# carlmoore256/MAAVSS

Measured on AMD Instinct MI355X. Metric: train clips/sec (16-frame×224² + 512-pt STFT) at 1/2/4/8 MI355X; mask-MSE vs ref, higher is better.
Workload: dtype f16; 1 GPU; batch=32/GPU, 16 frames 224x224, 512-pt STFT, ViT-S/8 attention extraction (f16 MFMA operands, f32 accumulate) + STFT + AV_Fusion_Model_Frames fwd+bwd (16-bit MFMA conv, f32 accumulate) + Adam; global_batch=32, frames=16, framesize=224, fft_len=512, parallelism=dp1, streams=2 (extraction of batch i+1 under the training step of batch i), avse_spatial_match=adaptive, vit_weights=random-init (no network), vit=f16, vit_gelu=f32, vit_qkv_ln=pre, vit_attention=f16, conv_fwd=f16, linear_lstm=f32 (split-K by f32 atomics), batchnorm=per-rank, grad_all_reduce=f32 wire, per-module buckets in backward order

## Files before the change

### include/maavss.h

```cpp
#ifndef MAAVSS_H
#define MAAVSS_H
#include <stdint.h>
#ifdef __cplusplus
extern "C" {
#endif

#define MAAVSS_ABI_VERSION 400
const char* maavss_last_error(void);
int maavss_version(void);
const char* maavss_arch(void);

int maavss_stft_fwd(const float* audio, int64_t batch, int64_t length, int64_t audio_stride, const float* window,
                    int n_fft, int hop, int n_frames, int n_bins_out, float* y, float* x, const float* noise,
                    float sigma, uint64_t seed, float* clip_absmax, void* stream);
int maavss_stft_normalise(float* y, float* x, const float* noise, const float* clip_absmax, int64_t batch,
                          int n_frames, int n_bins_out, float sigma, uint64_t seed, void* stream);

int maavss_istft(const float* spec, int64_t batch, int n_frames, int n_bins_in, const float* window, int n_fft, int hop,
                 int normalized, float* frames_ws, float* audio, int64_t audio_stride, void* stream);

int maavss_set_deterministic(int on);
int maavss_get_deterministic(void);
int maavss_set_deterministic_workspace(float* ws, int64_t bytes, void* stream);
int maavss_gemm_f32(const float* A, int64_t lda, int transA, const float* B, int64_t ldb, int transB, float* C,
// ... 114 lines not shown
int maavss_vit_patchify(const float* frames, void* a, int64_t n_frames, int H, int W, int dtype, void* stream);
int maavss_vit_gemm(const void* A, int lda, const void* W, const float* bias, const float* table, int period, void* C,
                    int ldc, int64_t M, int N, int K, int epilogue, int qscale_cols, float qscale, int dtype, void* stream);
int maavss_vit_layernorm(const float* x, const float* gamma, const float* beta, void* y, int64_t rows, int dim,
                         float eps, int dtype, void* stream);
int maavss_vit_panel_gemm(const float* X, const void* A, int lda, const float* ln_gamma, const float* ln_beta,
                          float ln_eps, const void* W, const float* bias, void* C, int ldc, int64_t c_rows, int64_t M,
                          int N, int epilogue, int qscale_cols, float qscale, int dtype, void* stream);
int maavss_vit_ws_gemm(const void* A, int lda, int64_t a_rows, const void* W, const float* bias, void* C, int ldc,
                       int64_t c_rows, int64_t M, int N, int epilogue, int qscale_cols, float qscale, void* xn_out,
                       const float* ln_gamma, const float* ln_beta, float ln_eps, int dtype, void* stream);
int maavss_vit_ws_gemm_ln(const float* X, int64_t x_rows, const float* row_stats, const float* ln_gamma, const float* ln_beta,
                          float ln_eps, const void* W, const float* bias, void* C, int ldc, int64_t c_rows, int64_t M, int N,
                          int qscale_cols, float qscale, int dtype, void* stream);
int maavss_vit_ws_gemm_ln_post(const float* X, int64_t x_rows, const float* row_stats, const float* col_sums, float ln_eps, const void* W,
                               const float* bias, void* C, int ldc, int64_t c_rows, int64_t M, int N, int qscale_cols, float qscale, int dtype,
                               void* stream);
int maavss_vit_gemm_stats(const void* A, int lda, const void* W, const float* bias, const float* table, int period, void* C,
                          int ldc, int64_t M, int N, int K, int epilogue, int qscale_cols, float qscale, float* row_stats,
                          int dtype, void* stream);
int maavss_vit_attn(const void* qkv, void* out, int frames, int ntok, int heads, int ld_qkv, int ld_out, int dtype,
                    void* stream);
int maavss_vit_cls_attn(const void* qkv, float* att, int frames, int ntok, int heads, int ld_qkv, int dtype, void* stream);
int64_t maavss_vit_attn_mx_ws_bytes(int64_t rows);
int maavss_vit_qkv_mx(const void* qkv, void* ws, int64_t rows, int ld_qkv, int dtype, void* stream);
int maavss_vit_attn_mx(const void* ws, void* out, int frames, int ntok, int heads, int ld_out, int dtype, void* stream);
int maavss_vit_ws_gemm_ln_mx(const float* X, int64_t x_rows, const float* row_stats, const float* ln_gamma, const float* ln_beta,
                             float ln_eps, const void* W, const float* bias, void* mx_ws, int64_t M, int qscale_cols, float qscale,
                             int dtype, void* stream);
int maavss_vit_attn_maps(const float* att, float* out, float* ws, int64_t n_frames, int heads, int H, int W,
                         int clip_frames, int attn_diff , void* stream);
int maavss_vit_attn_maps_checked(const float* att, float* out, float* ws, int64_t n_frames, int heads, int H, int W,
                                 int clip_frames, int attn_diff, int32_t* nonfinite_flag, void* stream);

int maavss_adaptive_pool_fwd(const float* x, float* out, int B, int H, int W, int C, int Ho, int Wo, int64_t os_b,
                             int64_t os_p, int64_t os_c, void* stream);
int maavss_adaptive_pool_bwd(const float* dout, float* dx, int B, int H, int W, int C, int Ho, int Wo, int64_t os_b,
                             int64_t os_p, int64_t os_c, void* stream);

int64_t maavss_video_transform_ws_bytes(int64_t F, int clip_frames, int H0, int W0, int S, int antialias, int autocontrast);
int maavss_video_transform(const void* src, const int32_t* boxes, const int32_t* host_boxes, float* out, void* ws, int64_t ws_bytes,
                           int64_t F, int clip_frames, int H0, int W0, int S, float mean0, float mean1, float mean2, float std0,
                           float std1, float std2, int antialias, int autocontrast, void* stream);

int maavss_vit_attn_maps_pass1(const float* att, float* small, float* fmax, int64_t n_frames, int heads, int n,
                               int32_t* nonfinite_flag, void* stream);
// ... 15 lines not shown
```

### maavss_amd/csrc/vit_attn.hip

```cpp
#include <type_traits>
#include "mma.h"

#define ATT_D 64
#define ATT_QT 128
#define ATT_KT 64
#define ATT_THR 5.0f
#ifdef MAAVSS_ATTN_ABLATE
#include <stdlib.h>
#define ABL(bit) ((ABLM >> (bit)) & 1)
#else
#define ABL(bit) 0
#endif

__device__ __forceinline__ float fast_exp2(float x) { return __builtin_amdgcn_exp2f(x); }

template <int MODE, int ABLM = 0>
__global__ __launch_bounds__(256) __attribute__((amdgpu_waves_per_eu(3, 3))) void vit_attn_kernel(
    const bf16_t* __restrict__ qkv, bf16_t* __restrict__ out, int ntok, int ld_qkv, int ld_out, int dim, int heads, int qblocks,
    int ngroups) {
  __shared__ __attribute__((aligned(16))) bf16_t Ks[2][ATT_KT * ATT_D];
  __shared__ __attribute__((aligned(16))) bf16_t Vs[2][ATT_KT * ATT_D];
  const int tid = threadIdx.x, lane = tid & 63, wv = tid >> 6, r = lane & 31, h = lane >> 5;
  const int xcd = blockIdx.x & 7, slot = blockIdx.x >> 3;
  const int group = (slot / qblocks) * 8 + xcd;
// ... 187 lines not shown
    if (last_half) tile(ntiles - 1, std::true_type{}, std::integral_constant<int, 1>{});
    else tile(ntiles - 1, std::true_type{}, std::integral_constant<int, 2>{});
  }
  {
    float la, lb;
    lane_swap32(lrow, la, lb);
    const float inv = 1.f / (la + lb);
    const int qr = q0 + r;
    if (qr < ntok) {
      bf16_t* op = out + (row0 + qr) * ld_out + head * ATT_D + 4 * h;
#pragma unroll
      for (int db = 0; db < 2; ++db)
#pragma unroll
        for (int g = 0; g < 4; ++g) {
          uint2 u;
          u.x = pack2<MODE>(o[db][4 * g] * inv, o[db][4 * g + 1] * inv);
          u.y = pack2<MODE>(o[db][4 * g + 2] * inv, o[db][4 * g + 3] * inv);
          *reinterpret_cast<uint2*>(op + 32 * db + 8 * g) = u;
        }
    }
  }
}

template <int MODE>
__global__ __launch_bounds__(256) void vit_cls_attn_kernel(const bf16_t* __restrict__ qkv, float* __restrict__ att, int ntok,
                                                           int ld_qkv, int dim) {
  extern __shared__ float sc[];
  __shared__ float qv[ATT_D];
  __shared__ float red[4];
  const int tid = threadIdx.x, head = blockIdx.x, frame = blockIdx.y;
  const int64_t row0 = (int64_t)frame * ntok;
  if (tid < ATT_D) qv[tid] = up16<MODE>(qkv[row0 * ld_qkv + head * ATT_D + tid]);
  __syncthreads();
  float mx = -1e30f;
  for (int j = tid; j < ntok; j += 256) {
    const bf16_t* kp = qkv + (row0 + j) * ld_qkv + dim + head * ATT_D;
    float acc = 0.f;
#pragma unroll
    for (int c = 0; c < 8; ++c) {
      const uint4 u = *reinterpret_cast<const uint4*>(kp + c * 8);
      const unsigned w[4] = {u.x, u.y, u.z, u.w};
#pragma unroll
      for (int e = 0; e < 4; ++e) {
        acc = fmaf(up16<MODE>((unsigned short)(w[e] & 0xffffu)), qv[c * 8 + 2 * e], acc);
        acc = fmaf(up16<MODE>((unsigned short)(w[e] >> 16)), qv[c * 8 + 2 * e + 1], acc);
      }
    }
    sc[j] = acc;
    mx = fmaxf(mx, acc);
  }
  mx = wave_max(mx);
  if ((tid & 63) == 0) red[tid >> 6] = mx;
  __syncthreads();
  mx = fmaxf(fmaxf(red[0], red[1]), fmaxf(red[2], red[3]));
  __syncthreads();
  float sum = 0.f;
  for (int j = tid; j < ntok; j += 256) {
    const float p = exp2f(sc[j] - mx);
    sc[j] = p;
    sum += p;
  }
  sum = wave_sum(sum);
  if ((tid & 63) == 0) red[tid >> 6] = sum;
  __syncthreads();
  const float inv = 1.f / (red[0] + red[1] + red[2] + red[3]);
  float* ap = att + ((int64_t)frame * gridDim.x + head) * (ntok - 1);
  for (int j = tid + 1; j < ntok; j += 256) ap[j - 1] = sc[j] * inv;
}

extern "C" int maavss_vit_attn(const void* qkv, void* out, int frames, int ntok, int heads, int ld_qkv, int ld_out, int dtype,
                               void* stream) {
  MAAVSS_CHECK_ARG(qkv && out && frames > 0 && ntok > 0, "vit_attn: bad arguments");
  MAAVSS_CHECK_ARG(heads >= 1 && ld_qkv >= 3 * heads * ATT_D && ld_out >= heads * ATT_D && ld_qkv % 8 == 0 && ld_out % 4 == 0,
                   "vit_attn: bad layout");
  MAAVSS_CHECK_ARG(dtype == MODE_BF16 || dtype == MODE_F16, "vit_attn: dtype must be 0 (bf16) or 2 (f16)");
  const int qblocks = cdiv(ntok, ATT_QT), ngroups = frames * heads;
  const int nblocks = cdiv(ngroups, 8) * 8 * qblocks;
  const bf16_t* q = (const bf16_t*)qkv;
  bf16_t* o = (bf16_t*)out;
  hipStream_t st = (hipStream_t)stream;
#ifdef MAAVSS_ATTN_ABLATE
  {
    const char* e = getenv("MAAVSS_ATTN_ABL");
    const int m = e ? atoi(e) : 0;
#define ABL_CASE(M) case M: hipLaunchKernelGGL((vit_attn_kernel<MODE_F16, M>), dim3(nblocks), dim3(256), 0, st, q, o, ntok, ld_qkv, ld_out, heads * ATT_D, heads, qblocks, ngroups); break;
    switch (m) { ABL_CASE(0) ABL_CASE(1) ABL_CASE(2) ABL_CASE(3) ABL_CASE(4) ABL_CASE(7) ABL_CASE(8) ABL_CASE(15) ABL_CASE(16) ABL_CASE(32) ABL_CASE(48) ABL_CASE(64) ABL_CASE(128) ABL_CASE(192) ABL_CASE(207) ABL_CASE(240)
      default: MAAVSS_CHECK_ARG(false, "vit_attn (ablation build): mask %d not instantiated", m); }
#undef ABL_CASE
    MAAVSS_LAUNCH_CHECK("vit_attn_kernel");
    return MAAVSS_OK;
  }
#endif
  if (dtype == MODE_F16)
    hipLaunchKernelGGL(vit_attn_kernel<MODE_F16>, dim3(nblocks), dim3(256), 0, st, q, o, ntok, ld_qkv, ld_out, heads * ATT_D, heads, qblocks, ngroups);
  else
    hipLaunchKernelGGL(vit_attn_kernel<MODE_BF16>, dim3(nblocks), dim3(256), 0, st, q, o, ntok, ld_qkv, ld_out, heads * ATT_D, heads, qblocks, ngroups);
  MAAVSS_LAUNCH_CHECK("vit_attn_kernel");
  return MAAVSS_OK;
}

extern "C" int maavss_vit_cls_attn(const void* qkv, float* att, int frames, int ntok, int heads, int ld_qkv, int dtype, void* stream) {
  MAAVSS_CHECK_ARG(qkv && att && frames > 0 && ntok > 1, "vit_cls_attn: bad arguments");
  MAAVSS_CHECK_ARG((size_t)ntok * 4 <= 60 * 1024, "vit_cls_attn: too many tokens for the LDS score buffer");
  MAAVSS_CHECK_ARG(dtype == MODE_BF16 || dtype == MODE_F16, "vit_cls_attn: dtype must be 0 (bf16) or 2 (f16)");
  if (dtype == MODE_F16)
    hipLaunchKernelGGL(vit_cls_attn_kernel<MODE_F16>, dim3(heads, frames), dim3(256), ntok * sizeof(float), (hipStream_t)stream,
                       (const bf16_t*)qkv, att, ntok, ld_qkv, heads * ATT_D);
  else
    hipLaunchKernelGGL(vit_cls_attn_kernel<MODE_BF16>, dim3(heads, frames), dim3(256), ntok * sizeof(float), (hipStream_t)stream,
                       (const bf16_t*)qkv, att, ntok, ld_qkv, heads * ATT_D);
  MAAVSS_LAUNCH_CHECK("vit_cls_attn_kernel");
  return MAAVSS_OK;
}
```

### maavss_amd/csrc/vit_ws_gemm.hip

```cpp
#include <type_traits>
#include <stdlib.h>
#include "mma.h"
#include "vit_epilogue.h"
#include "vit_mx.h"

#define WS_K 384
#define WS_BM 64
#define WS_WAVES 12
#define WS_THREADS (WS_WAVES * 64)
#define WS_SLICE (WS_WAVES * 32)
#define WS_BUFS 2
#define WS_PANEL_BYTES (WS_BM * WS_K * 2)

struct WsArgs {
  const bf16_t* A;
  const float* X;
  const float* row_stats;
  const bf16_t* W;
  const float* bias;
  void* C;
  bf16_t* XN;
  const float* ln_g;
  const float* ln_b;
  float ln_eps;
  int M, N, ldc;
  int qscale_cols;
  float qscale;
  int ns;
  int groups_per_xcd;
  int panels;
  MxImages mx;
};

#ifdef WS_STAMP
__device__ unsigned long long ws_stamps[256 * WS_WAVES * 8];
extern "C" int maavss_ws_stamps_read(unsigned long long* host, int clear) {
  if (hipMemcpyFromSymbol(host, HIP_SYMBOL(ws_stamps), sizeof(ws_stamps)) != hipSuccess) return 1;
  if (clear) { static unsigned long long z[256 * WS_WAVES * 8]; if (hipMemcpyToSymbol(HIP_SYMBOL(ws_stamps), z, sizeof(z)) != hipSuccess) return 1; }
  return 0;
}
#define WS_T(i) { const unsigned long long t_ = __builtin_amdgcn_s_memtime(); st_acc[i] += t_ - st_last; st_last = t_; }
#else
#define WS_T(i)
#endif

template <int EPI, int LN, int MODE, int SH>
__global__ __launch_bounds__(WS_THREADS) void vit_ws_gemm_kernel(WsArgs g) {
  static_assert(SH == 32 || SH == 16, "MFMA shape");
  static_assert(SH == 32 || EPI != 3, "the MX epilogue is built on the 32x32 accumulator layout");
  constexpr bool LN_POST = LN == 5;
  constexpr bool LN_OUT = LN == 1 || LN == 3, LN_IN = LN == 2 || LN == 4 || LN_POST, AFF = LN == 1 || LN == 2;
  static_assert(LN >= 0 && LN <= 5, "LN variant");
  static_assert(!LN_POST || (SH == 16 && EPI == 0), "LayerNorm after the product: 16x16x32 form, 16-bit epilogue");
  static_assert(!LN_OUT || EPI == 2, "LayerNorm of the output rows comes with the residual epilogue");
  static_assert(!LN_IN || EPI == 0 || EPI == 3, "LayerNorm on the way in is wired for the attn.qkv epilogues");
  static_assert(EPI != 3 || LN_IN, "the MX epilogue is wired for attn.qkv (LayerNorm on the way in)");
  extern __shared__ __attribute__((aligned(16))) char smem[];
  char* panels_lds = smem;
  float* bias_lds = reinterpret_cast<float*>(smem + WS_BUFS * WS_PANEL_BYTES);
  float* gam_lds = bias_lds + WS_SLICE;
  float* bet_lds = gam_lds + WS_SLICE;
  float2* stat_lds = reinterpret_cast<float2*>(bet_lds + WS_SLICE);
  const int tid = threadIdx.x, lane = tid & 63, wv = tid >> 6, r32 = lane & 31, half = lane >> 5;
  const int xcd = blockIdx.x & 7, slot = blockIdx.x >> 3;
  if (slot >= g.groups_per_xcd * g.ns) return;
  const int slice = slot % g.ns, group = xcd * g.groups_per_xcd + slot / g.ns, ngroups = 8 * g.groups_per_xcd;
  const int p0 = (int)((int64_t)g.panels * group / ngroups), p1 = (int)((int64_t)g.panels * (group + 1) / ngroups);
  if (p0 >= p1) return;
  const int n0 = slice * WS_SLICE + wv * 32;
#ifdef MAAVSS_WS_ABL
  constexpr int abl = MAAVSS_WS_ABL;
#else
  constexpr int abl = 0;
#endif

  typedef unsigned u32x4 __attribute__((ext_vector_type(4)));
  u32x4 stg0, stg1, stg2, stg3;
#define WS_FETCH(p)                                                                                               \
// ... 32 lines not shown
    int ln_ = lane;                                                                                               \
    asm volatile("" : "+v"(ln_));                                                                                 \
    char* dst_ = panels_lds + (buf) * WS_PANEL_BYTES;                                                             \
    WS_DEPOSIT_HALF_ONE(part, 0, stg0) WS_DEPOSIT_HALF_ONE(part, 1, stg1)                                         \
  }
  float4 st01;
  float2 st2;
#define WS_FETCH_X(hp, with_stats, srow)                                                                           \
  {                                                                                                               \
    const char* src_ = reinterpret_cast<const char*>(g.X) + (int64_t)(hp) * WS_PANEL_BYTES + (wv * 256 + lane) * 16; \
    if (with_stats) {                                                                                             \
      const char* sp_ = reinterpret_cast<const char*>(g.row_stats) + (int64_t)(srow) * 24;                         \
      asm volatile("global_load_dwordx4 %0, %6, off\n\tglobal_load_dwordx4 %1, %6, off offset:1024\n\t"            \
                   "global_load_dwordx4 %2, %6, off offset:2048\n\tglobal_load_dwordx4 %3, %6, off offset:3072\n\t" \
                   "global_load_dwordx4 %4, %7, off\n\tglobal_load_dwordx2 %5, %7, off offset:16"                  \
                   : "=&v"(stg0), "=&v"(stg1), "=&v"(stg2), "=&v"(stg3), "=&v"(st01), "=&v"(st2) : "v"(src_), "v"(sp_) : "memory"); \
    } else {                                                                                                      \
      asm volatile("global_load_dwordx4 %0, %4, off\n\tglobal_load_dwordx4 %1, %4, off offset:1024\n\t"            \
                   "global_load_dwordx4 %2, %4, off offset:2048\n\tglobal_load_dwordx4 %3, %4, off offset:3072"    \
                   : "=&v"(stg0), "=&v"(stg1), "=&v"(stg2), "=&v"(stg3) : "v"(src_) : "memory");                   \
    }                                                                                                             \
  }
  float2* table_lds = stat_lds;
  auto merge_stats = [&](const float4& a, const float2& b) __attribute__((always_inline)) {
    const float mean = (a.x + a.z + b.x) * (1.f / 3.f);
    const float d0 = a.x - mean, d1 = a.z - mean, d2 = b.x - mean;
    const float m2 = (a.y + a.w + b.y) + 128.f * (d0 * d0 + d1 * d1 + d2 * d2);
    return make_float2(mean, rsqrtf(m2 * (1.f / WS_K) + g.ln_eps));
  };
  auto deposit_ln_one = [&](char* dst, const float2* tab, int part, int i, const u32x4& raw, int ln) __attribute__((always_inline)) {
    const int q = (wv * 4 + i) * 64 + ln, r = q / 96, c4 = q - r * 96, rr = 32 * part + r;
    float2 ms = make_float2(0.f, 0.f);
    if constexpr (!LN_POST) ms = tab[rr];
    const float4 v = __builtin_bit_cast(float4, raw);
    uint2 o;
    if constexpr (LN_POST) {
      o = make_uint2(pack2<MODE>(v.x, v.y), pack2<MODE>(v.z, v.w));
    } else if constexpr (AFF) {
      const float4 gg = *reinterpret_cast<const float4*>(gam_lds + 4 * c4), bb = *reinterpret_cast<const float4*>(bet_lds + 4 * c4);
      o = make_uint2(pack2<MODE>((v.x - ms.x) * ms.y * gg.x + bb.x, (v.y - ms.x) * ms.y * gg.y + bb.y),
                     pack2<MODE>((v.z - ms.x) * ms.y * gg.z + bb.z, (v.w - ms.x) * ms.y * gg.w + bb.w));
    } else {
      o = make_uint2(pack2<MODE>((v.x - ms.x) * ms.y, (v.y - ms.x) * ms.y), pack2<MODE>((v.z - ms.x) * ms.y, (v.w - ms.x) * ms.y));
    }
    *reinterpret_cast<uint2*>(dst + rr * (WS_K * 2) + (((c4 >> 1) ^ (rr & 15)) << 4) + (c4 & 1) * 8) = o;
  };
#define WS_DEPOSIT_LN(buf, tab, part)                                                                             \
  {                                                                                                               \
    int ln_ = lane;                                                                                               \
    asm volatile("" : "+v"(ln_));                                                                                 \
    char* dst_ = panels_lds + (buf) * WS_PANEL_BYTES;                                                             \
    deposit_ln_one(dst_, tab, part, 0, stg0, ln_); deposit_ln_one(dst_, tab, part, 1, stg1, ln_);                 \
    deposit_ln_one(dst_, tab, part, 2, stg2, ln_); deposit_ln_one(dst_, tab, part, 3, stg3, ln_);                 \
  }
  constexpr bool SPLIT = EPI == 2;
  if constexpr (!LN_IN) WS_FETCH(p0)

#ifndef WS16_LN_SPLITCOLS
#define WS16_LN_SPLITCOLS 0
#endif
  constexpr bool F32OUT = EPI == 2 && (!LN_OUT || WS16_LN_SPLITCOLS);
  constexpr int CSTEP = F32OUT ? 16 : 4;
  const int j16 = lane & 15, g16 = lane >> 4;
  const int cbase16 = F32OUT ? 4 * g16 : 8 * g16;
  bf16x8 w[24];
  if constexpr (SH == 32) {
    const int q = r32 >> 3, h = (r32 >> 2) & 1, r = r32 & 3;
    const bf16_t* wp = g.W + (int64_t)(n0 + 16 * (q >> 1) + 8 * h + 4 * (q & 1) + r) * WS_K + 8 * half;
#pragma unroll
    for (int kb = 0; kb < 24; ++kb) w[kb] = *reinterpret_cast<const bf16x8*>(wp + kb * 16);
  } else {
#pragma unroll
    for (int b = 0; b < 2; ++b) {
      const int col = F32OUT ? 16 * b + j16 : 8 * (j16 >> 2) + 4 * b + (j16 & 3);
      const bf16_t* wp = g.W + (int64_t)(n0 + col) * WS_K + 8 * g16;
#pragma unroll
      for (int ks = 0; ks < 12; ++ks) w[12 * b + ks] = *reinterpret_cast<const bf16x8*>(wp + ks * 32);
    }
  }
  if (tid < WS_SLICE) {
    bias_lds[tid] = g.bias[slice * WS_SLICE + tid];
    if constexpr (AFF) { gam_lds[tid] = g.ln_g[tid]; bet_lds[tid] = g.ln_b[tid]; }
    if constexpr (LN_POST) gam_lds[tid] = g.ln_g[slice * WS_SLICE + tid];
  }
  if constexpr (!LN_IN) {
    WS_WAIT_FETCH(0)
    WS_DEPOSIT(0)
  } else {
    if (wv < 2 && p0 + wv < p1) {
      int row = (p0 + wv) * WS_BM + lane;
      row = row < g.M ? row : g.M - 1;
      const float* sp = g.row_stats + (int64_t)row * 6;
      table_lds[wv * WS_BM + lane] = merge_stats(*reinterpret_cast<const float4*>(sp), *reinterpret_cast<const float2*>(sp + 4));
    }
    __syncthreads();
#pragma unroll 1
    for (int part = 0; part < 2; ++part) {
      WS_FETCH_X(2 * p0 + part, false, 0)
      WS_WAIT_FETCH(0)
      WS_DEPOSIT_LN(0, table_lds, part)
    }
  }
  const int frag_r = r32 * (WS_K * 2) + ((half ^ (r32 & 1)) << 4), frag_x = (r32 & 14) << 4;
  const int frag16_r = j16 * (WS_K * 2) + ((g16 ^ (j16 & 3)) << 4), frag16_x = (j16 & 12) << 4;
  const float scale = ((EPI == 0 || EPI == 3) && slice * WS_SLICE < g.qscale_cols) ? g.qscale : 1.f;
  const bool vslice = EPI == 3 && slice == 2;

  constexpr int S = EPI == 2 ? (LN_OUT ? (SH == 16 && WS16_LN_SPLITCOLS ? 24 : 20) : 16) : 4;
  int it = 0;
#ifdef WS_STAMP
  unsigned long long st_acc[6] = {0, 0, 0, 0, 0, 0}, st_last = __builtin_amdgcn_s_memtime();
#endif
  for (int p = p0; p < p1; ++p, ++it) {
    const int buf = it & 1;
    asm volatile("s_waitcnt lgkmcnt(0)" ::: "memory");
    if (!(abl & 16)) __builtin_amdgcn_s_barrier();
    WS_T(0)
    const bool more = p + 1 < p1 && !((abl & 2) && it > 0);
    if constexpr (!SPLIT && !LN_IN) { if (more) WS_FETCH(p + 1) }
    const int m0 = p * WS_BM;
#pragma unroll 1
    for (int h2 = 0; h2 < 2; ++h2) {
      if constexpr (SPLIT) { if (more) WS_FETCH_HALF(p + 1, h2) }
      bool stats_next = false;
      if constexpr (LN_IN) {
        if (more) {
          stats_next = h2 == 0 && p + 2 < p1;
          int srow = (p + 2) * WS_BM + lane;
          srow = srow < g.M ? srow : g.M - 1;
          WS_FETCH_X(2 * (p + 1) + h2, stats_next, srow)
        }
// ... 27 lines not shown
        constexpr int D16 = LN == 4 ? 2 : LN_IN ? 1 : (EPI == 2) ? 2 : 3;
        {
          bf16x8 f[D16 + 1];
#pragma unroll
          for (int t = 0; t < D16; ++t) f[t] = rd16(t);
#pragma unroll
          for (int t = 0; t < 24; ++t) {
            if (t + D16 < 24 && !(abl & 8)) f[(t + D16) % (D16 + 1)] = rd16(t + D16);
            __builtin_amdgcn_sched_barrier(0);
            if (!(abl & 4)) {
              Mma<MODE>::mma(acc[t & 1][0], w[t >> 1], f[t % (D16 + 1)]);
              Mma<MODE>::mma(acc[t & 1][1], w[12 + (t >> 1)], f[t % (D16 + 1)]);
            } else if (t == 23) {
#pragma unroll
              for (int i = 0; i <= D16; ++i) acc[0][0][0] += (float)f[i][i];
            }
            __builtin_amdgcn_sched_barrier(0);
          }
        }
        WS_T(1)
        const int64_t row0 = m0 + 32 * h2 + j16;
        bool skip_epi16 = false;
        if constexpr ((abl & 1) != 0) skip_epi16 = acc[0][0][3] != 1234.5f;
        if (!skip_epi16) {
        if constexpr (EPI != 2) {
#pragma unroll
          for (int c = 0; c < 2; ++c) {
            bf16_t* cp = reinterpret_cast<bf16_t*>(g.C) + (row0 + 16 * c) * g.ldc + n0 + 8 * g16;
            v2f v[4] = {v2f{acc[c][0][0], acc[c][0][1]}, v2f{acc[c][0][2], acc[c][0][3]}, v2f{acc[c][1][0], acc[c][1][1]}, v2f{acc[c][1][2], acc[c][1][3]}};
            if constexpr (LN_POST) {
              int jj = lane;
              asm volatile("" : "+v"(jj));
              const float rs = table_lds[(it % 3) * WS_BM + 32 * h2 + 16 * c + (jj & 15)].y;
              const float* bp = bias_lds + (tid >> 6) * 32 + 8 * (jj >> 4);
              {
                const float4 b0 = *reinterpret_cast<const float4*>(bp);
                v[0].x = v[0].x * rs + b0.x; v[0].y = v[0].y * rs + b0.y; v[1].x = v[1].x * rs + b0.z; v[1].y = v[1].y * rs + b0.w;
              }
              {
                const float4 b1 = *reinterpret_cast<const float4*>(bp + 4);
                v[2].x = v[2].x * rs + b1.x; v[2].y = v[2].y * rs + b1.y; v[3].x = v[3].x * rs + b1.z; v[3].y = v[3].y * rs + b1.w;
              }
            }
            if constexpr (EPI == 4) {
              *reinterpret_cast<uint4*>(cp) = make_uint4(pg_gelu_h2(v[0]), pg_gelu_h2(v[1]), pg_gelu_h2(v[2]), pg_gelu_h2(v[3]));
              continue;
            } else if constexpr (EPI == 1) {
              pg_gelu4(v[0], v[1]);
              pg_gelu4(v[2], v[3]);
            } else {
#pragma unroll
              for (int e = 0; e < 4; ++e) { v[e].x *= scale; v[e].y *= scale; }
            }
            *reinterpret_cast<uint4*>(cp) = make_uint4(pack2<MODE>(v[0].x, v[0].y), pack2<MODE>(v[1].x, v[1].y),
                                                       pack2<MODE>(v[2].x, v[2].y), pack2<MODE>(v[3].x, v[3].y));
          }
        } else {
#pragma unroll
          for (int c = 0; c < 2; ++c) {
            float* cp = reinterpret_cast<float*>(g.C) + (row0 + 16 * c) * g.ldc + n0 + cbase16;
            const float4 x0 = *reinterpret_cast<const float4*>(cp), x1 = *reinterpret_cast<const float4*>(cp + CSTEP);
            acc[c][0][0] += x0.x; acc[c][0][1] += x0.y; acc[c][0][2] += x0.z; acc[c][0][3] += x0.w;
            acc[c][1][0] += x1.x; acc[c][1][1] += x1.y; acc[c][1][2] += x1.z; acc[c][1][3] += x1.w;
            *reinterpret_cast<float4*>(cp) = make_float4(acc[c][0][0], acc[c][0][1], acc[c][0][2], acc[c][0][3]);
            *reinterpret_cast<float4*>(cp + CSTEP) = make_float4(acc[c][1][0], acc[c][1][1], acc[c][1][2], acc[c][1][3]);
          }
          if constexpr (LN_OUT) {
            auto reduce2 = [&](float s0, float s1) __attribute__((always_inline)) {
              asm volatile("s_nop 1\n\tv_permlane16_swap_b32 %0, %1\n\ts_nop 1" : "+v"(s0), "+v"(s1));
              float ua, ub;
              lane_swap32(s0 + s1, ua, ub);
              return ua + ub;
            };
            const int cme = g16 & 1;
            float s0 = 0.f, s1 = 0.f;
#pragma unroll
            for (int b = 0; b < 2; ++b)
#pragma unroll
              for (int r = 0; r < 4; ++r) { s0 += acc[0][b][r]; s1 += acc[1][b][r]; }
            const float mu = reduce2(s0, s1) * (1.f / 32.f);
            float mu0, mu1;
            lane_swap16(mu, mu0, mu1);
            float q0 = 0.f, q1 = 0.f;
#pragma unroll
            for (int b = 0; b < 2; ++b)
#pragma unroll
              for (int r = 0; r < 4; ++r) {
                const float d0 = acc[0][b][r] - mu0, d1 = acc[1][b][r] - mu1;
                q0 += d0 * d0;
                q1 += d1 * d1;
              }
            const float m2 = reduce2(q0, q1);
            float2* sp = stat_lds + (32 * h2 + 16 * cme + j16);
            if (g16 < 2) sp[wv * WS_BM] = make_float2(mu, m2);
            asm volatile("s_waitcnt lgkmcnt(0)" ::: "memory");
            __builtin_amdgcn_s_barrier();
// ... 202 lines not shown
        }
      }
    }
    if constexpr (!SPLIT && !LN_IN) {
      if (more) {
        WS_WAIT_FETCH(S)
        WS_T(3)
        WS_DEPOSIT(buf ^ 1)
        WS_T(4)
      }
    }
  }
#ifdef WS_STAMP
  if (lane == 0) {
    unsigned long long* o = ws_stamps + ((size_t)blockIdx.x * WS_WAVES + wv) * 8;
    for (int i = 0; i < 5; ++i) o[i] = st_acc[i];
    o[5] = (unsigned long long)(p1 - p0);
  }
#endif
}

static int ws_gemm_launch(const char* who, const void* A, const float* X, const float* row_stats, const void* W, const float* bias,
                          void* C, int ldc, int64_t M, int N, int epilogue, int qscale_cols, float qscale, void* xn_out,
                          const float* ln_gamma, const float* ln_beta, float ln_eps, int dtype, void* stream, void* mx_ws = nullptr) {
  static int n_cu_dev[64] = {0};
  int dev = 0;
  MAAVSS_CHECK_ARG(hipGetDevice(&dev) == hipSuccess && dev >= 0 && dev < 64, "%s: cannot query the device", who);
  if (!n_cu_dev[dev]) {
    hipDeviceProp_t prop;
    MAAVSS_CHECK_ARG(hipGetDeviceProperties(&prop, dev) == hipSuccess, "%s: cannot query the device", who);
    n_cu_dev[dev] = prop.multiProcessorCount > 0 ? prop.multiProcessorCount : 256;
  }
  const int cu_per_xcd = n_cu_dev[dev] / 8 > 0 ? n_cu_dev[dev] / 8 : 1;
  WsArgs g;
  g.A = (const bf16_t*)A; g.X = X; g.row_stats = row_stats; g.W = (const bf16_t*)W; g.bias = bias; g.C = C; g.XN = (bf16_t*)xn_out;
  g.ln_g = ln_gamma; g.ln_b = ln_beta; g.ln_eps = ln_eps;
  g.M = (int)M; g.N = N; g.ldc = ldc; g.qscale_cols = qscale_cols; g.qscale = qscale;
  if (mx_ws) g.mx = mx_images(mx_ws, M);
  g.ns = N / WS_SLICE;
  MAAVSS_CHECK_ARG(g.ns <= cu_per_xcd, "%s: N too large for one XCD's CUs", who);
  g.groups_per_xcd = cu_per_xcd / g.ns;
  g.panels = cdiv(M, WS_BM);
  const size_t smem = WS_BUFS * WS_PANEL_BYTES + 3 * WS_SLICE * sizeof(float) + WS_BM * WS_WAVES * sizeof(float2);
  hipStream_t st = (hipStream_t)stream;
  const dim3 grid(8 * cu_per_xcd), block(WS_THREADS);
  static int shape_env = 0;
  if (!shape_env) {
    const char* e = getenv("MAAVSS_WS_SHAPE");
    shape_env = (e && e[0] == '3') ? 32 : 16;
  }
#define WS_LAUNCH4(E, L, D, H)                                                                                        \
  {                                                                                                                   \
    hipFuncSetAttribute(reinterpret_cast<const void*>(vit_ws_gemm_kernel<E, L, D, H>), hipFuncAttributeMaxDynamicSharedMemorySize, (int)smem); \
    hipLaunchKernelGGL((vit_ws_gemm_kernel<E, L, D, H>), grid, block, smem, st, g);                                   \
  }
#define WS_LAUNCH3(E, L, D) { if (shape_env == 32) WS_LAUNCH4(E, L, D, 32) else WS_LAUNCH4(E, L, D, 16) }
#define WS_LAUNCH(E, L) { if (dtype == MODE_F16) WS_LAUNCH3(E, L, MODE_F16) else WS_LAUNCH3(E, L, MODE_BF16) }
  const bool affine = ln_gamma != nullptr;
  if (X && epilogue == 3) {
    if (affine) { if (dtype == MODE_F16) WS_LAUNCH4(3, 2, MODE_F16, 32) else WS_LAUNCH4(3, 2, MODE_BF16, 32) }
    else { if (dtype == MODE_F16) WS_LAUNCH4(3, 4, MODE_F16, 32) else WS_LAUNCH4(3, 4, MODE_BF16, 32) }
  }
  else if (X && epilogue == 5) { if (dtype == MODE_F16) WS_LAUNCH4(0, 5, MODE_F16, 16) else WS_LAUNCH4(0, 5, MODE_BF16, 16) }
  else if (X && affine) WS_LAUNCH(0, 2) else if (X) WS_LAUNCH(0, 4) else if (epilogue == 0) WS_LAUNCH(0, 0) else if (epilogue == 1) WS_LAUNCH(1, 0)
  else if (epilogue == 4) WS_LAUNCH3(4, 0, MODE_F16) else if (xn_out && affine) WS_LAUNCH(2, 1) else if (xn_out) WS_LAUNCH(2, 3) else WS_LAUNCH(2, 0)
#undef WS_LAUNCH4
#undef WS_LAUNCH3
#undef WS_LAUNCH
  MAAVSS_LAUNCH_CHECK("vit_ws_gemm_kernel");
  return MAAVSS_OK;
}

extern "C" int maavss_vit_ws_gemm(const void* A, int lda, int64_t a_rows, const void* W, const float* bias, void* C, int ldc, int64_t c_rows,
                                  int64_t M, int N, int epilogue, int qscale_cols, float qscale, void* xn_out,
                                  const float* ln_gamma, const float* ln_beta, float ln_eps, int dtype, void* stream) {
  MAAVSS_CHECK_ARG(A && W && bias && C && M > 0 && M < (1LL << 31), "vit_ws_gemm: bad arguments");
  MAAVSS_CHECK_ARG(N % WS_SLICE == 0 && N >= WS_SLICE, "vit_ws_gemm: N must be a multiple of 384 (got %d)", N);
  MAAVSS_CHECK_ARG((epilogue >= 0 && epilogue <= 2) || epilogue == 4, "vit_ws_gemm: unknown epilogue");
  MAAVSS_CHECK_ARG(epilogue != 4 || dtype == MODE_F16, "vit_ws_gemm: epilogue 4 (GELU evaluated in packed half) needs the IEEE-half storage format (dtype 2)");
  MAAVSS_CHECK_ARG(dtype == MODE_BF16 || dtype == MODE_F16, "vit_ws_gemm: dtype must be 0 (bf16) or 2 (f16)");
  MAAVSS_CHECK_ARG(lda == WS_K, "vit_ws_gemm: A must be dense [rows][384] (lda = %d)", lda);
  MAAVSS_CHECK_ARG(a_rows >= (int64_t)cdiv(M, WS_BM) * WS_BM, "vit_ws_gemm: A needs ceil(M/64)*64 = %ld allocated rows (got %ld): whole panels are read",
                   (long)cdiv(M, WS_BM) * WS_BM, (long)a_rows);
  MAAVSS_CHECK_ARG(ldc % 8 == 0 && ldc >= N && qscale_cols % WS_SLICE == 0, "vit_ws_gemm: ldc must be a multiple of 8, qscale_cols a multiple of 384");
  MAAVSS_CHECK_ARG(c_rows >= (int64_t)cdiv(M, WS_BM) * WS_BM, "vit_ws_gemm: C needs ceil(M/64)*64 = %ld allocated rows (got %ld): stores are unguarded",
// ... 26 lines not shown
  MAAVSS_CHECK_ARG(N % WS_SLICE == 0 && N >= WS_SLICE, "vit_ws_gemm_ln_post: N must be a multiple of 384 (got %d)", N);
  MAAVSS_CHECK_ARG(dtype == MODE_BF16 || dtype == MODE_F16, "vit_ws_gemm_ln_post: dtype must be 0 (bf16) or 2 (f16)");
  MAAVSS_CHECK_ARG(x_rows >= (int64_t)cdiv(M, WS_BM) * WS_BM && c_rows >= (int64_t)cdiv(M, WS_BM) * WS_BM,
                   "vit_ws_gemm_ln_post: X and C need ceil(M/64)*64 = %ld allocated rows (got %ld, %ld): whole panels are read and stored",
                   (long)cdiv(M, WS_BM) * WS_BM, (long)x_rows, (long)c_rows);
  MAAVSS_CHECK_ARG(ldc % 8 == 0 && ldc >= N && qscale_cols % WS_SLICE == 0, "vit_ws_gemm_ln_post: ldc must be a multiple of 8, qscale_cols a multiple of 384");
  return ws_gemm_launch("vit_ws_gemm_ln_post", nullptr, X, row_stats, W, bias, C, ldc, M, N, 5, qscale_cols, qscale, nullptr, col_sums, nullptr, ln_eps,
                        dtype, stream);
}

extern "C" int maavss_vit_ws_gemm_ln_mx(const float* X, int64_t x_rows, const float* row_stats, const float* ln_gamma, const float* ln_beta,
                                        float ln_eps, const void* W, const float* bias, void* mx_ws, int64_t M, int qscale_cols, float qscale,
                                        int dtype, void* stream) {
  MAAVSS_CHECK_ARG(X && row_stats && W && bias && mx_ws && M > 0 && M < (1LL << 31), "vit_ws_gemm_ln_mx: bad arguments");
  MAAVSS_CHECK_ARG((ln_gamma != nullptr) == (ln_beta != nullptr), "vit_ws_gemm_ln_mx: ln_gamma / ln_beta both given or both null (null = no affine part)");
  MAAVSS_CHECK_ARG(dtype == MODE_BF16 || dtype == MODE_F16, "vit_ws_gemm_ln_mx: dtype (of the weights) must be 0 (bf16) or 2 (f16)");
  MAAVSS_CHECK_ARG(x_rows >= (int64_t)cdiv(M, WS_BM) * WS_BM, "vit_ws_gemm_ln_mx: X needs ceil(M/64)*64 = %ld allocated rows (got %ld): whole panels are read",
                   (long)cdiv(M, WS_BM) * WS_BM, (long)x_rows);
  MAAVSS_CHECK_ARG(qscale_cols % WS_SLICE == 0 && ((uintptr_t)mx_ws & 255) == 0, "vit_ws_gemm_ln_mx: qscale_cols must be a multiple of 384, mx_ws 256-byte aligned");
  MAAVSS_CHECK_ARG(mx_ws_bytes(M) < (1LL << 32), "vit_ws_gemm_ln_mx: %ld rows: workspace beyond the attention kernel's 32-bit offsets (launch fewer frames per group)", (long)M);
  return ws_gemm_launch("vit_ws_gemm_ln_mx", nullptr, X, row_stats, W, bias, mx_ws, 3 * WS_SLICE, M, 3 * WS_SLICE, 3, qscale_cols, qscale, nullptr,
                        ln_gamma, ln_beta, ln_eps, dtype, stream, mx_ws);
}
```

### maavss_amd/video_attention.py

```python
import math
import os
import sys
from typing import NamedTuple

import torch

from . import _lib
from ._lib import call, ptr, stream_ptr

DIM, DEPTH, HEADS, MLP, PATCH = 384, 12, 6, 1536, 8
LN_EPS = 1e-6
EPI_BF16_BIAS, EPI_BF16_BIAS_GELU, EPI_F32_BIAS_RESID, EPI_F32_ROWTABLE = 0, 1, 2, 3
DT_BF16, DT_F16 = 0, 2
_TORCH_DT = {DT_BF16: torch.bfloat16, DT_F16: torch.float16}


class ViTSpec(NamedTuple):
    dim: int
    heads: int
    mlp: int
    depth: int
    checkpoint: str


# ... 218 lines not shown
        qkv = torch.empty(rpad, 3 * DIM, device=dev, dtype=tdt)
        att_o = torch.empty(rpad, DIM, device=dev, dtype=tdt)
        hid = torch.empty(rpad, MLP, device=dev, dtype=tdt)
        ws8 = None
        if self.attn_fp8:
            key = (rows, torch.cuda.current_stream().cuda_stream)
            ws8 = self._mx_ws.pop(key, None)
            if ws8 is None:
                while len(self._mx_ws) >= 4:
                    self._mx_ws.pop(next(iter(self._mx_ws)))
                ws8 = torch.zeros(_lib.query("maavss_vit_attn_mx_ws_bytes", rows), device=dev, dtype=torch.uint8)
            self._mx_ws[key] = ws8
            x[rows:].zero_()
            att_o[rows:].zero_()
        call("maavss_vit_patchify", ptr(frames), ptr(a), f, h, w, dt, st)
        call("maavss_vit_gemm_stats", ptr(a), 192, ptr(wts["patch_w"]), None, ptr(table), ntok, ptr(x), DIM, rows, DIM, 192,
             EPI_F32_ROWTABLE, 0, 1.0, ptr(stats) if (self.ws_gemm and self.ws_ln_in) else None, dt, st)
        qs = 0.125 * 1.4426950408889634
        for i in range(DEPTH):
            b = wts[i]
            nqkv = 2 * DIM if i == DEPTH - 1 else 3 * DIM
            fp8_here = self.attn_fp8 and i in self.fp8_blocks
            mx_fused = fp8_here and self.ws_gemm and self.ws_ln_in and i < DEPTH - 1
            if mx_fused:
                call("maavss_vit_ws_gemm_ln_mx", ptr(x), rpad, ptr(stats), ptr(b["n1w"]), ptr(b["n1b"]), LN_EPS, ptr(b["qkv_w"]),
                     ptr(b["qkv_b"]), ptr(ws8), rows, DIM, qs, dt, st)
            elif self.ws_gemm:
                if not self.ws_ln_in:
                    call("maavss_vit_layernorm", ptr(x), ptr(b["n1w"]), ptr(b["n1b"]), ptr(xn), rows, DIM, LN_EPS, dt, st)
                    call("maavss_vit_ws_gemm", ptr(xn), DIM, rpad, ptr(b["qkv_w"]), ptr(b["qkv_b"]), ptr(qkv), 3 * DIM, rpad, rows, nqkv,
                         EPI_BF16_BIAS, DIM, qs, None, None, None, LN_EPS, dt, st)
                else:
                  if self.qkv_ln == "post":
                      call("maavss_vit_ws_gemm_ln_post", ptr(x), rpad, ptr(stats), ptr(b["qkv_cs"]), LN_EPS, ptr(b["qkv_wf"]), ptr(b["qkv_bf"]),
                           ptr(qkv), 3 * DIM, rpad, rows, nqkv, DIM, qs, dt, st)
                  else:
                      call("maavss_vit_ws_gemm_ln", ptr(x), rpad, ptr(stats), ptr(b["n1w"]), ptr(b["n1b"]), LN_EPS, ptr(b["qkv_w"]),
                           ptr(b["qkv_b"]), ptr(qkv), 3 * DIM, rpad, rows, nqkv, DIM, qs, dt, st)
            elif self.fused_panel_gemm:
                call("maavss_vit_panel_gemm", ptr(x), None, 0, ptr(b["n1w"]), ptr(b["n1b"]), LN_EPS, ptr(b["qkv_w"]),
                     ptr(b["qkv_b"]), ptr(qkv), 3 * DIM, rpad, rows, nqkv, EPI_BF16_BIAS, DIM, qs, dt, st)
            else:
                call("maavss_vit_layernorm", ptr(x), ptr(b["n1w"]), ptr(b["n1b"]), ptr(xn), rows, DIM, LN_EPS, dt, st)
                call("maavss_vit_gemm", ptr(xn), DIM, ptr(b["qkv_w"]), ptr(b["qkv_b"]), None, 0, ptr(qkv), 3 * DIM, rows,
                     nqkv, DIM, EPI_BF16_BIAS, DIM, qs, dt, st)
            if i == DEPTH - 1:
# ... 123 lines not shown
```

Baseline: 839.5 clips/s.

## Fuse last-block key projection with CLS scores to skip full QKV

```diff
diff --git a/include/maavss.h b/include/maavss.h
--- a/include/maavss.h
+++ b/include/maavss.h
@@ -160,6 +160,11 @@
 int maavss_vit_attn(const void* qkv, void* out, int frames, int ntok, int heads, int ld_qkv, int ld_out, int dtype,
                     void* stream);
 int maavss_vit_cls_attn(const void* qkv, float* att, int frames, int ntok, int heads, int ld_qkv, int dtype, void* stream);
+int maavss_vit_cls_rows(const float* X, const float* row_stats, float* Xc, float* stats_c, int frames, int ntok, void* stream);
+int maavss_vit_ws_gemm_ln_score(const float* X, int64_t x_rows, const float* row_stats, const float* ln_gamma, const float* ln_beta,
+                                float ln_eps, const void* Wk, const float* bias_k, const void* qcls, float* scores, int64_t score_rows,
+                                int64_t M, int ntok, int dtype, void* stream);
+int maavss_vit_cls_softmax(const float* scores, int64_t score_rows, float* att, int frames, int ntok, int heads, void* stream);
 int64_t maavss_vit_attn_mx_ws_bytes(int64_t rows);
 int maavss_vit_qkv_mx(const void* qkv, void* ws, int64_t rows, int ld_qkv, int dtype, void* stream);
 int maavss_vit_attn_mx(const void* ws, void* out, int frames, int ntok, int heads, int ld_out, int dtype, void* stream);
diff --git a/maavss_amd/csrc/vit_attn.hip b/maavss_amd/csrc/vit_attn.hip
--- a/maavss_amd/csrc/vit_attn.hip
+++ b/maavss_amd/csrc/vit_attn.hip
@@ -233,6 +233,26 @@
   }
 }
 
+__device__ __forceinline__ void cls_softmax_store(float* sc, float mx, int ntok, float* __restrict__ ap, float* red) {
+  const int tid = threadIdx.x;
+  mx = wave_max(mx);
+  if ((tid & 63) == 0) red[tid >> 6] = mx;
+  __syncthreads();
+  mx = fmaxf(fmaxf(red[0], red[1]), fmaxf(red[2], red[3]));
+  __syncthreads();
+  float sum = 0.f;
+  for (int j = tid; j < ntok; j += 256) {
+    const float p = exp2f(sc[j] - mx);
+    sc[j] = p;
+    sum += p;
+  }
+  sum = wave_sum(sum);
+  if ((tid & 63) == 0) red[tid >> 6] = sum;
+  __syncthreads();
+  const float inv = 1.f / (red[0] + red[1] + red[2] + red[3]);
+  for (int j = tid + 1; j < ntok; j += 256) ap[j - 1] = sc[j] * inv;
+}
+
 template <int MODE>
 __global__ __launch_bounds__(256) void vit_cls_attn_kernel(const bf16_t* __restrict__ qkv, float* __restrict__ att, int ntok,
                                                            int ld_qkv, int dim) {
@@ -260,23 +280,21 @@
     sc[j] = acc;
     mx = fmaxf(mx, acc);
   }
-  mx = wave_max(mx);
-  if ((tid & 63) == 0) red[tid >> 6] = mx;
-  __syncthreads();
-  mx = fmaxf(fmaxf(red[0], red[1]), fmaxf(red[2], red[3]));
-  __syncthreads();
-  float sum = 0.f;
+  cls_softmax_store(sc, mx, ntok, att + ((int64_t)frame * gridDim.x + head) * (ntok - 1), red);
+}
+
+__global__ __launch_bounds__(256) void vit_cls_softmax_kernel(const float* __restrict__ scores, int64_t ld, float* __restrict__ att, int ntok) {
+  extern __shared__ float sc[];
+  __shared__ float red[4];
+  const int tid = threadIdx.x, head = blockIdx.x, frame = blockIdx.y;
+  const float* lo = scores + (int64_t)(2 * head) * ld + (int64_t)frame * ntok;
+  float mx = -1e30f;
   for (int j = tid; j < ntok; j += 256) {
-    const float p = exp2f(sc[j] - mx);
-    sc[j] = p;
-    sum += p;
-  }
-  sum = wave_sum(sum);
-  if ((tid & 63) == 0) red[tid >> 6] = sum;
-  __syncthreads();
-  const float inv = 1.f / (red[0] + red[1] + red[2] + red[3]);
-  float* ap = att + ((int64_t)frame * gridDim.x + head) * (ntok - 1);
-  for (int j = tid + 1; j < ntok; j += 256) ap[j - 1] = sc[j] * inv;
+    const float s = lo[j] + lo[ld + j];
+    sc[j] = s;
+    mx = fmaxf(mx, s);
+  }
+  cls_softmax_store(sc, mx, ntok, att + ((int64_t)frame * gridDim.x + head) * (ntok - 1), red);
 }
 
 extern "C" int maavss_vit_attn(const void* qkv, void* out, int frames, int ntok, int heads, int ld_qkv, int ld_out, int dtype,
@@ -323,3 +341,12 @@
   MAAVSS_LAUNCH_CHECK("vit_cls_attn_kernel");
   return MAAVSS_OK;
 }
+
+extern "C" int maavss_vit_cls_softmax(const float* scores, int64_t score_rows, float* att, int frames, int ntok, int heads, void* stream) {
+  MAAVSS_CHECK_ARG(scores && att && frames > 0 && ntok > 1 && heads >= 1, "vit_cls_softmax: bad arguments");
+  MAAVSS_CHECK_ARG(score_rows >= (int64_t)frames * ntok, "vit_cls_softmax: %ld score rows allocated for %d frames of %d tokens", (long)score_rows, frames, ntok);
+  MAAVSS_CHECK_ARG((size_t)ntok * 4 <= 60 * 1024, "vit_cls_softmax: too many tokens for the LDS score buffer");
+  hipLaunchKernelGGL(vit_cls_softmax_kernel, dim3(heads, frames), dim3(256), ntok * sizeof(float), (hipStream_t)stream, scores, score_rows, att, ntok);
+  MAAVSS_LAUNCH_CHECK("vit_cls_softmax_kernel");
+  return MAAVSS_OK;
+}
diff --git a/maavss_amd/csrc/vit_ws_gemm.hip b/maavss_amd/csrc/vit_ws_gemm.hip
--- a/maavss_amd/csrc/vit_ws_gemm.hip
+++ b/maavss_amd/csrc/vit_ws_gemm.hip
@@ -19,6 +19,8 @@
   const bf16_t* W;
   const float* bias;
   void* C;
+  const bf16_t* qcls;
+  unsigned ntok_magic, ntok_shift;
   bf16_t* XN;
   const float* ln_g;
   const float* ln_b;
@@ -44,6 +46,14 @@
 #define WS_T(i)
 #endif
 
+__device__ __forceinline__ float2 ws_merge_stats(const float4& a, const float2& b, float eps) {
+  const float mean = (a.x + a.z + b.x) * (1.f / 3.f);
+  const float d0 = a.x - mean, d1 = a.z - mean, d2 = b.x - mean;
+  const float m2 = (a.y + a.w + b.y) + 128.f * (d0 * d0 + d1 * d1 + d2 * d2);
+  return make_float2(mean, rsqrtf(m2 * (1.f / WS_K) + eps));
+}
+__device__ __forceinline__ float ws_ln_affine(float v, const float2& ms, float gam, float bet) { return (v - ms.x) * ms.y * gam + bet; }
+
 template <int EPI, int LN, int MODE, int SH>
 __global__ __launch_bounds__(WS_THREADS) void vit_ws_gemm_kernel(WsArgs g) {
   static_assert(SH == 32 || SH == 16, "MFMA shape");
@@ -53,7 +63,8 @@
   static_assert(LN >= 0 && LN <= 5, "LN variant");
   static_assert(!LN_POST || (SH == 16 && EPI == 0), "LayerNorm after the product: 16x16x32 form, 16-bit epilogue");
   static_assert(!LN_OUT || EPI == 2, "LayerNorm of the output rows comes with the residual epilogue");
-  static_assert(!LN_IN || EPI == 0 || EPI == 3, "LayerNorm on the way in is wired for the attn.qkv epilogues");
+  static_assert(!LN_IN || EPI == 0 || EPI == 3 || EPI == 6, "LayerNorm on the way in is wired for the attn.qkv epilogues");
+  static_assert(EPI != 6 || (LN == 2 && SH == 16), "the CLS-score epilogue is built on the 16x16 accumulator layout with norm1 on the way in");
   static_assert(EPI != 3 || LN_IN, "the MX epilogue is wired for attn.qkv (LayerNorm on the way in)");
   extern __shared__ __attribute__((aligned(16))) char smem[];
   char* panels_lds = smem;
@@ -132,12 +143,7 @@
     }                                                                                                             \
   }
   float2* table_lds = stat_lds;
-  auto merge_stats = [&](const float4& a, const float2& b) __attribute__((always_inline)) {
-    const float mean = (a.x + a.z + b.x) * (1.f / 3.f);
-    const float d0 = a.x - mean, d1 = a.z - mean, d2 = b.x - mean;
-    const float m2 = (a.y + a.w + b.y) + 128.f * (d0 * d0 + d1 * d1 + d2 * d2);
-    return make_float2(mean, rsqrtf(m2 * (1.f / WS_K) + g.ln_eps));
-  };
+  auto merge_stats = [&](const float4& a, const float2& b) __attribute__((always_inline)) { return ws_merge_stats(a, b, g.ln_eps); };
   auto deposit_ln_one = [&](char* dst, const float2* tab, int part, int i, const u32x4& raw, int ln) __attribute__((always_inline)) {
     const int q = (wv * 4 + i) * 64 + ln, r = q / 96, c4 = q - r * 96, rr = 32 * part + r;
     float2 ms = make_float2(0.f, 0.f);
@@ -148,8 +154,8 @@
       o = make_uint2(pack2<MODE>(v.x, v.y), pack2<MODE>(v.z, v.w));
     } else if constexpr (AFF) {
       const float4 gg = *reinterpret_cast<const float4*>(gam_lds + 4 * c4), bb = *reinterpret_cast<const float4*>(bet_lds + 4 * c4);
-      o = make_uint2(pack2<MODE>((v.x - ms.x) * ms.y * gg.x + bb.x, (v.y - ms.x) * ms.y * gg.y + bb.y),
-                     pack2<MODE>((v.z - ms.x) * ms.y * gg.z + bb.z, (v.w - ms.x) * ms.y * gg.w + bb.w));
+      o = make_uint2(pack2<MODE>(ws_ln_affine(v.x, ms, gg.x, bb.x), ws_ln_affine(v.y, ms, gg.y, bb.y)),
+                     pack2<MODE>(ws_ln_affine(v.z, ms, gg.z, bb.z), ws_ln_affine(v.w, ms, gg.w, bb.w)));
     } else {
       o = make_uint2(pack2<MODE>((v.x - ms.x) * ms.y, (v.y - ms.x) * ms.y), pack2<MODE>((v.z - ms.x) * ms.y, (v.w - ms.x) * ms.y));
     }
@@ -187,6 +193,10 @@
 #pragma unroll
       for (int ks = 0; ks < 12; ++ks) w[12 * b + ks] = *reinterpret_cast<const bf16x8*>(wp + ks * 32);
     }
+  }
+  if constexpr (EPI == 6) {
+#pragma unroll
+    for (int kb = 0; kb < 24; ++kb) asm volatile("" ::"v"(w[kb]));
   }
   if (tid < WS_SLICE) {
     bias_lds[tid] = g.bias[slice * WS_SLICE + tid];
@@ -216,7 +226,7 @@
   const float scale = ((EPI == 0 || EPI == 3) && slice * WS_SLICE < g.qscale_cols) ? g.qscale : 1.f;
   const bool vslice = EPI == 3 && slice == 2;
 
-  constexpr int S = EPI == 2 ? (LN_OUT ? (SH == 16 && WS16_LN_SPLITCOLS ? 24 : 20) : 16) : 4;
+  constexpr int S = EPI == 2 ? (LN_OUT ? (SH == 16 && WS16_LN_SPLITCOLS ? 24 : 20) : 16) : EPI == 6 ? 6 : 4;
   int it = 0;
 #ifdef WS_STAMP
   unsigned long long st_acc[6] = {0, 0, 0, 0, 0, 0}, st_last = __builtin_amdgcn_s_memtime();
@@ -290,8 +300,41 @@
         const int64_t row0 = m0 + 32 * h2 + j16;
         bool skip_epi16 = false;
         if constexpr ((abl & 1) != 0) skip_epi16 = acc[0][0][3] != 1234.5f;
+        auto reduce2 = [&](float s0, float s1) __attribute__((always_inline)) {
+          asm volatile("s_nop 1\n\tv_permlane16_swap_b32 %0, %1\n\ts_nop 1" : "+v"(s0), "+v"(s1));
+          float ua, ub;
+          lane_swap32(s0 + s1, ua, ub);
+          return ua + ub;
+        };
         if (!skip_epi16) {
-        if constexpr (EPI != 2) {
+        if constexpr (EPI == 6) {
+          int to = tid;
+          asm volatile("" : "+v"(to));
+          const int jo = to & 15, go = (to >> 4) & 3, rowo = m0 + 32 * h2 + jo;
+          uint4 qv[2];
+#pragma unroll
+          for (int c = 0; c < 2; ++c) {
+            const int rc = rowo + 16 * c < g.M ? rowo + 16 * c : g.M - 1;
+            const unsigned frame = __umulhi((unsigned)rc, g.ntok_magic) >> g.ntok_shift;
+            qv[c] = *reinterpret_cast<const uint4*>(g.qcls + (int64_t)frame * WS_K + (to >> 6) * 32 + 8 * go);
+          }
+          float sc[2];
+#pragma unroll
+          for (int c = 0; c < 2; ++c) {
+            const unsigned kk[4] = {pack2<MODE>(acc[c][0][0], acc[c][0][1]), pack2<MODE>(acc[c][0][2], acc[c][0][3]),
+                                    pack2<MODE>(acc[c][1][0], acc[c][1][1]), pack2<MODE>(acc[c][1][2], acc[c][1][3])};
+            const unsigned qq[4] = {qv[c].x, qv[c].y, qv[c].z, qv[c].w};
+            float a = 0.f;
+#pragma unroll
+            for (int e = 0; e < 4; ++e) {
+              a = fmaf(up16<MODE>((unsigned short)(kk[e] & 0xffffu)), up16<MODE>((unsigned short)(qq[e] & 0xffffu)), a);
+              a = fmaf(up16<MODE>((unsigned short)(kk[e] >> 16)), up16<MODE>((unsigned short)(qq[e] >> 16)), a);
+            }
+            sc[c] = a;
+          }
+          const float tot = reduce2(sc[0], sc[1]);
+          if (go < 2) reinterpret_cast<float*>(g.C)[(int64_t)(to >> 6) * g.ldc + rowo + 16 * go] = tot;
+        } else if constexpr (EPI != 2) {
 #pragma unroll
           for (int c = 0; c < 2; ++c) {
             bf16_t* cp = reinterpret_cast<bf16_t*>(g.C) + (row0 + 16 * c) * g.ldc + n0 + 8 * g16;
@@ -334,12 +377,6 @@
             *reinterpret_cast<float4*>(cp + CSTEP) = make_float4(acc[c][1][0], acc[c][1][1], acc[c][1][2], acc[c][1][3]);
           }
           if constexpr (LN_OUT) {
-            auto reduce2 = [&](float s0, float s1) __attribute__((always_inline)) {
-              asm volatile("s_nop 1\n\tv_permlane16_swap_b32 %0, %1\n\ts_nop 1" : "+v"(s0), "+v"(s1));
-              float ua, ub;
-              lane_swap32(s0 + s1, ua, ub);
-              return ua + ub;
-            };
             const int cme = g16 & 1;
             float s0 = 0.f, s1 = 0.f;
 #pragma unroll
@@ -588,7 +625,8 @@
 
 static int ws_gemm_launch(const char* who, const void* A, const float* X, const float* row_stats, const void* W, const float* bias,
                           void* C, int ldc, int64_t M, int N, int epilogue, int qscale_cols, float qscale, void* xn_out,
-                          const float* ln_gamma, const float* ln_beta, float ln_eps, int dtype, void* stream, void* mx_ws = nullptr) {
+                          const float* ln_gamma, const float* ln_beta, float ln_eps, int dtype, void* stream, void* mx_ws = nullptr,
+                          const void* qcls = nullptr, int ntok = 1) {
   static int n_cu_dev[64] = {0};
   int dev = 0;
   MAAVSS_CHECK_ARG(hipGetDevice(&dev) == hipSuccess && dev >= 0 && dev < 64, "%s: cannot query the device", who);
@@ -602,6 +640,13 @@
   g.A = (const bf16_t*)A; g.X = X; g.row_stats = row_stats; g.W = (const bf16_t*)W; g.bias = bias; g.C = C; g.XN = (bf16_t*)xn_out;
   g.ln_g = ln_gamma; g.ln_b = ln_beta; g.ln_eps = ln_eps;
   g.M = (int)M; g.N = N; g.ldc = ldc; g.qscale_cols = qscale_cols; g.qscale = qscale;
+  g.qcls = (const bf16_t*)qcls;
+  {
+    int L = 0;
+    while ((1LL << L) < ntok) ++L;
+    g.ntok_magic = (unsigned)(((1ULL << (31 + L)) + ntok - 1) / ntok);
+    g.ntok_shift = L > 0 ? L - 1 : 0;
+  }
   if (mx_ws) g.mx = mx_images(mx_ws, M);
   g.ns = N / WS_SLICE;
   MAAVSS_CHECK_ARG(g.ns <= cu_per_xcd, "%s: N too large for one XCD's CUs", who);
@@ -627,6 +672,7 @@
     if (affine) { if (dtype == MODE_F16) WS_LAUNCH4(3, 2, MODE_F16, 32) else WS_LAUNCH4(3, 2, MODE_BF16, 32) }
     else { if (dtype == MODE_F16) WS_LAUNCH4(3, 4, MODE_F16, 32) else WS_LAUNCH4(3, 4, MODE_BF16, 32) }
   }
+  else if (X && epilogue == 6) { if (dtype == MODE_F16) WS_LAUNCH4(6, 2, MODE_F16, 16) else WS_LAUNCH4(6, 2, MODE_BF16, 16) }
   else if (X && epilogue == 5) { if (dtype == MODE_F16) WS_LAUNCH4(0, 5, MODE_F16, 16) else WS_LAUNCH4(0, 5, MODE_BF16, 16) }
   else if (X && affine) WS_LAUNCH(0, 2) else if (X) WS_LAUNCH(0, 4) else if (epilogue == 0) WS_LAUNCH(0, 0) else if (epilogue == 1) WS_LAUNCH(1, 0)
   else if (epilogue == 4) WS_LAUNCH3(4, 0, MODE_F16) else if (xn_out && affine) WS_LAUNCH(2, 1) else if (xn_out) WS_LAUNCH(2, 3) else WS_LAUNCH(2, 0)
@@ -699,3 +745,31 @@
   return ws_gemm_launch("vit_ws_gemm_ln_mx", nullptr, X, row_stats, W, bias, mx_ws, 3 * WS_SLICE, M, 3 * WS_SLICE, 3, qscale_cols, qscale, nullptr,
                         ln_gamma, ln_beta, ln_eps, dtype, stream, mx_ws);
 }
+
+__global__ __launch_bounds__(WS_K / 4) void vit_cls_rows_kernel(const float* __restrict__ X, const float* __restrict__ row_stats, float* __restrict__ Xc,
+                                                                float* __restrict__ stats_c, int ntok) {
+  const int f = blockIdx.x, t = threadIdx.x;
+  const int64_t row = (int64_t)f * ntok;
+  reinterpret_cast<float4*>(Xc + (int64_t)f * WS_K)[t] = reinterpret_cast<const float4*>(X + row * WS_K)[t];
+  if (t < 6) stats_c[f * 6 + t] = row_stats[row * 6 + t];
+}
+
+extern "C" int maavss_vit_cls_rows(const float* X, const float* row_stats, float* Xc, float* stats_c, int frames, int ntok, void* stream) {
+  MAAVSS_CHECK_ARG(X && row_stats && Xc && stats_c && frames > 0 && ntok > 0, "vit_cls_rows: bad arguments");
+  hipLaunchKernelGGL(vit_cls_rows_kernel, dim3(frames), dim3(WS_K / 4), 0, (hipStream_t)stream, X, row_stats, Xc, stats_c, ntok);
+  MAAVSS_LAUNCH_CHECK("vit_cls_rows_kernel");
+  return MAAVSS_OK;
+}
+
+extern "C" int maavss_vit_ws_gemm_ln_score(const float* X, int64_t x_rows, const float* row_stats, const float* ln_gamma, const float* ln_beta,
+                                           float ln_eps, const void* Wk, const float* bias_k, const void* qcls, float* scores, int64_t score_rows,
+                                           int64_t M, int ntok, int dtype, void* stream) {
+  MAAVSS_CHECK_ARG(X && row_stats && ln_gamma && ln_beta && Wk && bias_k && qcls && scores && M > 0 && M < (1LL << 31), "vit_ws_gemm_ln_score: bad arguments");
+  MAAVSS_CHECK_ARG(ntok > 1 && M % ntok == 0, "vit_ws_gemm_ln_score: M (%ld) must be whole frames of ntok = %d rows", (long)M, ntok);
+  MAAVSS_CHECK_ARG(dtype == MODE_BF16 || dtype == MODE_F16, "vit_ws_gemm_ln_score: dtype must be 0 (bf16) or 2 (f16)");
+  MAAVSS_CHECK_ARG(x_rows >= (int64_t)cdiv(M, WS_BM) * WS_BM && score_rows >= (int64_t)cdiv(M, WS_BM) * WS_BM && score_rows < (1LL << 31),
+                   "vit_ws_gemm_ln_score: X and scores need ceil(M/64)*64 = %ld allocated rows (got %ld, %ld): whole panels are read and stored",
+                   (long)cdiv(M, WS_BM) * WS_BM, (long)x_rows, (long)score_rows);
+  return ws_gemm_launch("vit_ws_gemm_ln_score", nullptr, X, row_stats, Wk, bias_k, scores, (int)score_rows, M, WS_SLICE, 6, 0, 1.f, nullptr, ln_gamma,
+                        ln_beta, ln_eps, dtype, stream, nullptr, qcls, ntok);
+}
diff --git a/maavss_amd/video_attention.py b/maavss_amd/video_attention.py
--- a/maavss_amd/video_attention.py
+++ b/maavss_amd/video_attention.py
@@ -264,6 +264,20 @@
             nqkv = 2 * DIM if i == DEPTH - 1 else 3 * DIM
             fp8_here = self.attn_fp8 and i in self.fp8_blocks
             mx_fused = fp8_here and self.ws_gemm and self.ws_ln_in and i < DEPTH - 1
+            if i == DEPTH - 1 and self.ws_gemm and self.ws_ln_in and self.qkv_ln == "pre":
+                fpad = (f + 63) // 64 * 64
+                xc = torch.empty(fpad, DIM, device=dev, dtype=torch.float32)
+                stats_c = torch.empty(f, 3, 2, device=dev, dtype=torch.float32)
+                qcls = torch.empty(fpad, DIM, device=dev, dtype=tdt)
+                scores = torch.empty(2 * HEADS, rpad, device=dev, dtype=torch.float32)
+                att = torch.empty(f, HEADS, ntok - 1, device=dev, dtype=torch.float32)
+                call("maavss_vit_cls_rows", ptr(x), ptr(stats), ptr(xc), ptr(stats_c), f, ntok, st)
+                call("maavss_vit_ws_gemm_ln", ptr(xc), fpad, ptr(stats_c), ptr(b["n1w"]), ptr(b["n1b"]), LN_EPS, ptr(b["qkv_w"]), ptr(b["qkv_b"]),
+                     ptr(qcls), DIM, fpad, f, DIM, DIM, qs, dt, st)
+                call("maavss_vit_ws_gemm_ln_score", ptr(x), rpad, ptr(stats), ptr(b["n1w"]), ptr(b["n1b"]), LN_EPS, ptr(b["qkv_w"][DIM:2 * DIM]),
+                     ptr(b["qkv_b"][DIM:2 * DIM]), ptr(qcls), ptr(scores), rpad, rows, ntok, dt, st)
+                call("maavss_vit_cls_softmax", ptr(scores), rpad, ptr(att), f, ntok, HEADS, st)
+                return att
             if mx_fused:
                 call("maavss_vit_ws_gemm_ln_mx", ptr(x), rpad, ptr(stats), ptr(b["n1w"]), ptr(b["n1b"]), LN_EPS, ptr(b["qkv_w"]),
                      ptr(b["qkv_b"]), ptr(ws8), rows, DIM, qs, dt, st)
```

New measurement: 845.4 clips/s, median of 6. Within noise of the previous version (+0.7%).
